# scaomath/galerkin-transformer

Measured on AMD Instinct MI355X. Metric: training samples/s, Darcy 141x141 Galerkin encoder (fwd+loss+bwd+clip+Adam), higher is better.
Workload: dtype f32 (operands split into 2 fp16 terms under a running per-row / per-tile power-of-two scale, 3 products on the f16 MFMA pipe, f32 accumulate; fp32-class results: the 1e-5 parity suite passes in this mode; packed-B token GEMMs, convolutions, weight gradients, regression head and the Fourier attention

## Files before the change

galerkin-transformer_amd/csrc/gt_head.hip:

```cpp
#include "gt_common.h"
#include <algorithm>

namespace gt {

constexpr int HK = 32, HN = 128;
constexpr int W1P = 36;
constexpr int DHP = 68;
constexpr int HSLAB = HN * HK + 2 * HN + 1;

struct HeadP {
    const float* X; const float* W1; const float* b1; const float* w2; const float* b2; const float* g;
    float* out; float* dX; float* slabs;
    int64_t T;
    int n_mtiles;
    const float* gate = nullptr;
};

__device__ __forceinline__ void head_gate4(const float* gp, f32x4& v) {
    const f32x4 gt = *reinterpret_cast<const f32x4*>(gp);
#pragma unroll
    for (int t = 0; t < 4; ++t) v[t] *= dsilu_f(gt[t]);
}

template <int ACT>
__device__ __forceinline__ void head_act(float h, float& a, float& da) {
    if (ACT == GT_ACT_SILU) silu_both(h, a, da);
    else if (ACT == GT_ACT_RELU) { a = fmaxf(h, 0.f); da = h > 0.f ? 1.f : 0.f; }
    else { a = h; da = 1.f; }
}

__device__ __forceinline__ void head_stage_weights(const HeadP& p, float* sW1, float* sB1, float* sW2) {
    const int tid = threadIdx.x;
    for (int e = tid; e < HN * HK; e += 256) sW1[(e >> 5) * W1P + (e & 31)] = p.W1[e];
    if (tid < HN) {
        sB1[tid] = p.b1 ? p.b1[tid] : 0.f;
        sW2[tid] = p.w2[tid];
    }
    __syncthreads();
}

template <int NMT>
__device__ __forceinline__ void head_gemm1(const float* sW1, int hb, int j, int kq, const float (&xs)[8],
                                           f32x4 (&acc)[NMT]) {
#pragma unroll
    for (int mt = 0; mt < NMT; mt += 2) {
        f32x4 w[2][2];
#pragma unroll
        for (int u = 0; u < 2; ++u) {
            w[u][0] = *reinterpret_cast<const f32x4*>(&sW1[(hb + 16 * (mt + u) + j) * W1P + 8 * kq]);
            w[u][1] = *reinterpret_cast<const f32x4*>(&sW1[(hb + 16 * (mt + u) + j) * W1P + 8 * kq + 4]);
            acc[mt + u] = f32x4{0.f, 0.f, 0.f, 0.f};
        }
#pragma unroll
        for (int s = 0; s < 8; ++s)
#pragma unroll
            for (int u = 0; u < 2; ++u)
                acc[mt + u] = __builtin_amdgcn_mfma_f32_16x16x4f32(w[u][s >> 2][s & 3], xs[s], acc[mt + u], 0, 0, 0);
    }
}

template <int ACT>
__global__ __launch_bounds__(256, 2) void head_fwd_kernel(const HeadP p) {
    __shared__ __attribute__((aligned(16))) float sW1[HN * W1P];
    __shared__ __attribute__((aligned(16))) float sB1[HN], sW2[HN];
    const int lane = threadIdx.x & 63, wave = threadIdx.x >> 6;
    const int j = lane & 15, kq = lane >> 4;
    head_stage_weights(p, sW1, sB1, sW2);
    const float b2v = p.b2 ? p.b2[0] : 0.f;
    const int stride = gridDim.x * 4;
    int mtile = blockIdx.x * 4 + wave;
    f32x4 xa = {0.f, 0.f, 0.f, 0.f}, xb = {0.f, 0.f, 0.f, 0.f};
    if (mtile < p.n_mtiles) {
        const int64_t row = std::min<int64_t>((int64_t)mtile * 16 + j, p.T - 1);
        xa = *reinterpret_cast<const f32x4*>(p.X + row * HK + 8 * kq);
        xb = *reinterpret_cast<const f32x4*>(p.X + row * HK + 8 * kq + 4);
    }
    for (; mtile < p.n_mtiles; mtile += stride) {
        const int64_t m0 = (int64_t)mtile * 16;
        const float xs[8] = {xa[0], xa[1], xa[2], xa[3], xb[0], xb[1], xb[2], xb[3]};
        if (mtile + stride < p.n_mtiles) {
            const int64_t row = std::min<int64_t>((int64_t)(mtile + stride) * 16 + j, p.T - 1);
            xa = *reinterpret_cast<const f32x4*>(p.X + row * HK + 8 * kq);
            xb = *reinterpret_cast<const f32x4*>(p.X + row * HK + 8 * kq + 4);
        }
        f32x4 acc[8];
        head_gemm1<8>(sW1, 0, j, kq, xs, acc);
        float part = 0.f;
#pragma unroll
        for (int mt = 0; mt < 8; ++mt) {
            const f32x4 bv = *reinterpret_cast<const f32x4*>(&sB1[16 * mt + 4 * kq]);
            const f32x4 wv = *reinterpret_cast<const f32x4*>(&sW2[16 * mt + 4 * kq]);
#pragma unroll
            for (int r = 0; r < 4; ++r) {
                float a, da;
                head_act<ACT>(acc[mt][r] + bv[r], a, da);
                part = fmaf(a, wv[r], part);
            }
        }
        part += __shfl_xor(part, 16, 64);
        part += __shfl_xor(part, 32, 64);
        if (kq == 0 && m0 + j < p.T) p.out[m0 + j] = part + b2v;
    }
}

template <int ACT>
__global__ __launch_bounds__(256, 2) void head_bwd_kernel(const HeadP p) {
    __shared__ __attribute__((aligned(16))) float sW1[HN * W1P];
    __shared__ __attribute__((aligned(16))) float sB1[HN], sW2[HN];
    __shared__ __attribute__((aligned(16))) float sScr[4 * 16 * DHP + 2 * 4 * 2 * 256];
    const int tid = threadIdx.x, lane = tid & 63, wave = tid >> 6;
    const int j = lane & 15, kq = lane >> 4;
    const int pair = wave >> 1, half = wave & 1, hb = 64 * half;
    head_stage_weights(p, sW1, sB1, sW2);
    float* dh = sScr + wave * 16 * DHP;
    float* exch = sScr + 4 * 16 * DHP;

    f32x4 accW[4][2], sumW2[4], sumB1[4];
    float gsum = 0.f;
#pragma unroll
    for (int mt = 0; mt < 4; ++mt) {
        accW[mt][0] = accW[mt][1] = f32x4{0.f, 0.f, 0.f, 0.f};
        sumW2[mt] = sumB1[mt] = f32x4{0.f, 0.f, 0.f, 0.f};
    }
    const int stride = gridDim.x * 2;
    const int first = blockIdx.x * 2;
    const int iters = first < p.n_mtiles ? (p.n_mtiles - 1 - first) / stride + 1 : 0;
    int mtile = first + pair;
    f32x4 xa = {0.f, 0.f, 0.f, 0.f}, xb = {0.f, 0.f, 0.f, 0.f};
    float gv = 0.f;
    if (mtile < p.n_mtiles) {
        const int64_t nrow = (int64_t)mtile * 16 + j, row = std::min<int64_t>(nrow, p.T - 1);
        xa = *reinterpret_cast<const f32x4*>(p.X + row * HK + 8 * kq);
        xb = *reinterpret_cast<const f32x4*>(p.X + row * HK + 8 * kq + 4);
        gv = (nrow < p.T) ? p.g[row] : 0.f;
    }
    for (int it = 0; it < iters; ++it, mtile += stride) {
        const bool active = mtile < p.n_mtiles;
        const int64_t m0 = (int64_t)mtile * 16;
        const float xs[8] = {xa[0], xa[1], xa[2], xa[3], xb[0], xb[1], xb[2], xb[3]};
        const float g = active ? gv : 0.f;
        if (mtile + stride < p.n_mtiles) {
            const int64_t nrow = (int64_t)(mtile + stride) * 16 + j, row = std::min<int64_t>(nrow, p.T - 1);
            xa = *reinterpret_cast<const f32x4*>(p.X + row * HK + 8 * kq);
            xb = *reinterpret_cast<const f32x4*>(p.X + row * HK + 8 * kq + 4);
            gv = (nrow < p.T) ? p.g[row] : 0.f;
        }
        float* ex = exch + (it & 1) * (4 * 2 * 256);
        f32x4 acc[4];
        f32x4 accX[2] = {{0.f, 0.f, 0.f, 0.f}, {0.f, 0.f, 0.f, 0.f}};
        if (active) {
            head_gemm1<4>(sW1, hb, j, kq, xs, acc);
            gsum += (kq == 0 && half == 0) ? g : 0.f;
#pragma unroll
            for (int mt = 0; mt < 4; ++mt) {
                const f32x4 bv = *reinterpret_cast<const f32x4*>(&sB1[hb + 16 * mt + 4 * kq]);
                const f32x4 wv = *reinterpret_cast<const f32x4*>(&sW2[hb + 16 * mt + 4 * kq]);
#pragma unroll
                for (int r = 0; r < 4; ++r) {
                    float a, da;
                    head_act<ACT>(acc[mt][r] + bv[r], a, da);
                    const float d = g * wv[r] * da;
                    sumW2[mt][r] = fmaf(g, a, sumW2[mt][r]);
                    sumB1[mt][r] += d;
                    acc[mt][r] = d;
                }
                *reinterpret_cast<f32x4*>(&dh[j * DHP + 16 * mt + 4 * kq]) = acc[mt];
            }
#pragma unroll
            for (int mt = 0; mt < 4; ++mt)
#pragma unroll
                for (int s = 0; s < 4; ++s)
#pragma unroll
                    for (int t = 0; t < 2; ++t)
                        accX[t] = __builtin_amdgcn_mfma_f32_16x16x4f32(
                            sW1[(hb + 16 * mt + 4 * kq + s) * W1P + 16 * t + j], acc[mt][s], accX[t], 0, 0, 0);
        }
        *reinterpret_cast<f32x4*>(&ex[(wave * 2 + (half ^ 1)) * 256 + lane * 4]) = accX[half ^ 1];
        __syncthreads();
        if (active) {
            if (p.dX && m0 + j < p.T) {
                const f32x4 o = *reinterpret_cast<const f32x4*>(&ex[((wave ^ 1) * 2 + half) * 256 + lane * 4]);
                f32x4 dxv = accX[half] + o;
                if (p.gate) head_gate4(p.gate + (m0 + j) * HK + 16 * half + 4 * kq, dxv);
                *reinterpret_cast<f32x4*>(p.dX + (m0 + j) * HK + 16 * half + 4 * kq) = dxv;
            }
            float xr[2][4];
#pragma unroll
            for (int s = 0; s < 4; ++s) {
                const int64_t row = std::min<int64_t>(m0 + 4 * kq + s, p.T - 1);
#pragma unroll
                for (int t = 0; t < 2; ++t) xr[t][s] = p.X[row * HK + 16 * t + j];
            }
#pragma unroll
            for (int mt = 0; mt < 4; ++mt)
#pragma unroll
                for (int s = 0; s < 4; ++s) {
                    const float a = dh[(4 * kq + s) * DHP + 16 * mt + j];
#pragma unroll
                    for (int t = 0; t < 2; ++t)
                        accW[mt][t] = __builtin_amdgcn_mfma_f32_16x16x4f32(a, xr[t][s], accW[mt][t], 0, 0, 0);
                }
        }
    }
#pragma unroll
    for (int mt = 0; mt < 4; ++mt)
#pragma unroll
        for (int r = 0; r < 4; ++r) {
            float a = sumW2[mt][r], b = sumB1[mt][r];
#pragma unroll
            for (int o = 1; o < 16; o <<= 1) {
                a += __shfl_xor(a, o, 64);
                b += __shfl_xor(b, o, 64);
            }
            sumW2[mt][r] = a;
            sumB1[mt][r] = b;
        }
#pragma unroll
    for (int o = 1; o < 16; o <<= 1) gsum += __shfl_xor(gsum, o, 64);
    __syncthreads();
    float* red = sScr;
    for (int w = 0; w < 4; ++w) {
        if (wave == w) {
            const bool init = w < 2;
#pragma unroll
            for (int mt = 0; mt < 4; ++mt) {
#pragma unroll
                for (int t = 0; t < 2; ++t)
#pragma unroll
                    for (int r = 0; r < 4; ++r) {
                        float* q = &red[(hb + 16 * mt + 4 * kq + r) * HK + 16 * t + j];
                        *q = init ? accW[mt][t][r] : *q + accW[mt][t][r];
                    }
                if (j == 0) {
#pragma unroll
                    for (int r = 0; r < 4; ++r) {
                        float* q2 = &red[HN * HK + hb + 16 * mt + 4 * kq + r];
                        float* q1 = &red[HN * HK + HN + hb + 16 * mt + 4 * kq + r];
                        *q2 = init ? sumW2[mt][r] : *q2 + sumW2[mt][r];
                        *q1 = init ? sumB1[mt][r] : *q1 + sumB1[mt][r];
                    }
                }
            }
            if (lane == 0 && half == 0) {
                float* q = &red[HN * HK + 2 * HN];
                *q = (w == 0) ? gsum : *q + gsum;
            }
        }
        __syncthreads();
    }
    float* out = p.slabs + (int64_t)blockIdx.x * HSLAB;
    for (int e = tid; e < HSLAB; e += 256) out[e] = red[e];
}

__global__ __launch_bounds__(256) void head_reduce_kernel(const float* __restrict__ slabs, int nslab, float* dW1,
                                                         float* dw2, float* db1, float* db2) {
    __shared__ float part[8][32];
    const int el = threadIdx.x & 31, sl = threadIdx.x >> 5;
    const int e = blockIdx.x * 32 + el;
    float a0 = 0.f, a1 = 0.f;
    if (e < HSLAB) {
        int s = sl;
        for (; s + 8 < nslab; s += 16) {
            a0 += slabs[(int64_t)s * HSLAB + e];
            a1 += slabs[(int64_t)(s + 8) * HSLAB + e];
        }
        if (s < nslab) a0 += slabs[(int64_t)s * HSLAB + e];
    }
    part[sl][el] = a0 + a1;
    __syncthreads();
    if (sl != 0 || e >= HSLAB) return;
    float v = part[0][el];
#pragma unroll
    for (int k = 1; k < 8; ++k) v += part[k][el];
    if (e < HN * HK) dW1[e] = v;
    else if (e < HN * HK + HN) { if (dw2) dw2[e - HN * HK] = v; }
    else if (e < HN * HK + 2 * HN) { if (db1) db1[e - HN * HK - HN] = v; }
    else if (db2) db2[0] = v;
}

typedef _Float16 hf16x8 __attribute__((ext_vector_type(8)));
typedef _Float16 hf16x2 __attribute__((ext_vector_type(2)));
typedef uint32_t hu32x4 __attribute__((ext_vector_type(4)));

__device__ __forceinline__ int h16_exp_for(float amax) {
    const int ex = (int)(__float_as_uint(amax) >> 23);
    return ex == 0 ? 0 : (141 - ex > 126 ? 126 : 141 - ex);
}
__device__ __forceinline__ void h16_split_pair(float a, float b, float s, uint32_t& hi, uint32_t& lo) {
    const f32x2 r = f32x2{a, b} * s;
    const hf16x2 h0 = __builtin_convertvector(r, hf16x2);
    const hf16x2 h1 = __builtin_convertvector(r - __builtin_convertvector(h0, f32x2), hf16x2);
    hi = __builtin_bit_cast(uint32_t, h0);
    lo = __builtin_bit_cast(uint32_t, h1);
}
__device__ __forceinline__ void h16_split8(const float (&v)[8], float s, hf16x8& hi, hf16x8& lo) {
    uint32_t h[4], l[4];
#pragma unroll
    for (int t = 0; t < 4; ++t) h16_split_pair(v[2 * t], v[2 * t + 1], s, h[t], l[t]);
    hi = __builtin_bit_cast(hf16x8, hu32x4{h[0], h[1], h[2], h[3]});
    lo = __builtin_bit_cast(hf16x8, hu32x4{l[0], l[1], l[2], l[3]});
}
__device__ __forceinline__ f32x4 h16_mma3(hf16x8 ah, hf16x8 al, hf16x8 bh, hf16x8 bl, f32x4 acc) {
    acc = __builtin_amdgcn_mfma_f32_16x16x32_f16(al, bh, acc, 0, 0, 0);
    acc = __builtin_amdgcn_mfma_f32_16x16x32_f16(ah, bl, acc, 0, 0, 0);
    return __builtin_amdgcn_mfma_f32_16x16x32_f16(ah, bh, acc, 0, 0, 0);
}

template <bool WT>
__device__ __forceinline__ int head16_stage(const HeadP& p, hu32x4* sW1, hu32x4* sWT, float* sB1, float* sW2, float* sRed) {
    const int tid = threadIdx.x, lane = tid & 63, wave = tid >> 6;
    float v[2][8], m = 0.f;
#pragma unroll
    for (int u = 0; u < 2; ++u) {
        const int f = tid + 256 * u, mt = f >> 6, j = f & 15, kq = (f & 63) >> 4;
        const f32x4 a = *reinterpret_cast<const f32x4*>(p.W1 + (16 * mt + j) * HK + 8 * kq);
        const f32x4 b = *reinterpret_cast<const f32x4*>(p.W1 + (16 * mt + j) * HK + 8 * kq + 4);
#pragma unroll
        for (int e = 0; e < 4; ++e) {
            v[u][e] = a[e];
            v[u][4 + e] = b[e];
            m = fmaxf(m, fmaxf(fabsf(a[e]), fabsf(b[e])));
        }
    }
#pragma unroll
    for (int o = 32; o > 0; o >>= 1) m = fmaxf(m, __shfl_xor(m, o, 64));
    if (lane == 0) sRed[wave] = m;
    if (tid < HN) {
        sB1[tid] = p.b1 ? p.b1[tid] : 0.f;
        sW2[tid] = p.w2[tid];
    }
    __syncthreads();
    const int eW = h16_exp_for(fmaxf(fmaxf(sRed[0], sRed[1]), fmaxf(sRed[2], sRed[3])));
    const float sw = pow2_clamped(eW);
#pragma unroll
    for (int u = 0; u < 2; ++u) {
        hf16x8 hi, lo;
        h16_split8(v[u], sw, hi, lo);
        sW1[tid + 256 * u] = __builtin_bit_cast(hu32x4, hi);
        sW1[512 + tid + 256 * u] = __builtin_bit_cast(hu32x4, lo);
    }
    if (WT) {
#pragma unroll
        for (int u = 0; u < 2; ++u) {
            const int f = tid + 256 * u, t = f >> 7, ti = (f >> 6) & 1, mm = f & 15, kq = (f & 63) >> 4;
            float w[8];
#pragma unroll
            for (int e = 0; e < 8; ++e) w[e] = p.W1[(32 * t + 16 * (e >> 2) + 4 * kq + (e & 3)) * HK + 16 * ti + mm];
            hf16x8 hi, lo;
            h16_split8(w, sw, hi, lo);
            sWT[f] = __builtin_bit_cast(hu32x4, hi);
            sWT[512 + f] = __builtin_bit_cast(hu32x4, lo);
        }
    }
    __syncthreads();
    return eW;
}

__device__ __forceinline__ int head16_split_row(const float (&xs)[8], hf16x8& xh, hf16x8& xl) {
    float m = 0.f;
#pragma unroll
    for (int e = 0; e < 8; ++e) m = fmaxf(m, fabsf(xs[e]));
    m = fmaxf(m, __shfl_xor(m, 16, 64));
    m = fmaxf(m, __shfl_xor(m, 32, 64));
    const int ex = h16_exp_for(m);
    h16_split8(xs, pow2_clamped(ex), xh, xl);
    return ex;
}

template <int ACT>
__global__ __launch_bounds__(256, 2) void head_fwd16_kernel(const HeadP p) {
    __shared__ hu32x4 sW1[2 * 512];
    __shared__ __attribute__((aligned(16))) float sB1[HN], sW2[HN];
    __shared__ float sRed[4];
    const int lane = threadIdx.x & 63, wave = threadIdx.x >> 6;
    const int j = lane & 15, kq = lane >> 4;
    const int eW = head16_stage<false>(p, sW1, nullptr, sB1, sW2, sRed);
    const float b2v = p.b2 ? p.b2[0] : 0.f;
    const int stride = gridDim.x * 4;
    int mtile = blockIdx.x * 4 + wave;
    f32x4 xa = {0.f, 0.f, 0.f, 0.f}, xb = {0.f, 0.f, 0.f, 0.f};
    if (mtile < p.n_mtiles) {
        const int64_t row = std::min<int64_t>((int64_t)mtile * 16 + j, p.T - 1);
        xa = *reinterpret_cast<const f32x4*>(p.X + row * HK + 8 * kq);
        xb = *reinterpret_cast<const f32x4*>(p.X + row * HK + 8 * kq + 4);
    }
    for (; mtile < p.n_mtiles; mtile += stride) {
        const int64_t m0 = (int64_t)mtile * 16;
        const float xs[8] = {xa[0], xa[1], xa[2], xa[3], xb[0], xb[1], xb[2], xb[3]};
        if (mtile + stride < p.n_mtiles) {
            const int64_t row = std::min<int64_t>((int64_t)(mtile + stride) * 16 + j, p.T - 1);
            xa = *reinterpret_cast<const f32x4*>(p.X + row * HK + 8 * kq);
            xb = *reinterpret_cast<const f32x4*>(p.X + row * HK + 8 * kq + 4);
        }
        hf16x8 xh, xl;
        const int ex = head16_split_row(xs, xh, xl);
        const float us = pow2_clamped(-ex) * pow2_clamped(-eW);
        float part = 0.f;
#pragma unroll
        for (int mt = 0; mt < 8; ++mt) {
            const hf16x8 wh = __builtin_bit_cast(hf16x8, sW1[mt * 64 + lane]);
            const hf16x8 wl = __builtin_bit_cast(hf16x8, sW1[512 + mt * 64 + lane]);
            const f32x4 acc = h16_mma3(wh, wl, xh, xl, f32x4{0.f, 0.f, 0.f, 0.f});
            const f32x4 bv = *reinterpret_cast<const f32x4*>(&sB1[16 * mt + 4 * kq]);
            const f32x4 wv = *reinterpret_cast<const f32x4*>(&sW2[16 * mt + 4 * kq]);
#pragma unroll
            for (int r = 0; r < 4; ++r) {
                float a, da;
                head_act<ACT>(fmaf(acc[r], us, bv[r]), a, da);
                part = fmaf(a, wv[r], part);
            }
        }
        part += __shfl_xor(part, 16, 64);
        part += __shfl_xor(part, 32, 64);
        if (kq == 0 && m0 + j < p.T) p.out[m0 + j] = part + b2v;
    }
}

constexpr int DH16P = 68;
constexpr int H16_LIMIT = 15, H16_TARGET = 13;
constexpr int H16_SMEM = 4 * 512 * 16 + (2 * HN + 16) * 4 + 4 * 32 * DH16P * 4 + 4 * 32 * 4 + 4 * 2 * 256 * 4;

template <int ACT>
__global__ __launch_bounds__(256, 2) void head_bwd16_kernel(const HeadP p) {
    extern __shared__ __attribute__((aligned(16))) char hsm[];
    hu32x4* sW1 = reinterpret_cast<hu32x4*>(hsm);
    hu32x4* sWT = sW1 + 1024;
    float* sB1 = reinterpret_cast<float*>(sWT + 1024);
    float* sW2 = sB1 + HN;
    float* sRed = sW2 + HN;
    float* sDh = sRed + 16;
    float* sF = sDh + 4 * 32 * DH16P;
    float* sEx = sF + 4 * 32;
    const int tid = threadIdx.x, lane = tid & 63, wave = tid >> 6;
    const int j = lane & 15, kq = lane >> 4;
    const int pair = wave >> 1, half = wave & 1, hb = 64 * half;
    const int eW = head16_stage<true>(p, sW1, sWT, sB1, sW2, sRed);
    const float usW = pow2_clamped(-eW);
    float* dh = sDh + wave * 32 * DH16P;
    float* fr = sF + wave * 32;

    f32x4 accW[4][2], sumW2[4], sumB1[4];
    float gsum = 0.f;
#pragma unroll
    for (int mt = 0; mt < 4; ++mt) {
        accW[mt][0] = accW[mt][1] = f32x4{0.f, 0.f, 0.f, 0.f};
        sumW2[mt] = sumB1[mt] = f32x4{0.f, 0.f, 0.f, 0.f};
    }
    int cexp = 100;
    const int n32 = (int)((p.T + 31) / 32);
    const int stride = gridDim.x * 2;
    const int first = blockIdx.x * 2;
    const int iters = first < n32 ? (n32 - 1 - first) / stride + 1 : 0;
    int tile = first + pair;
    f32x4 xa[2], xb[2];
    float gv[2];
    auto load = [&](int tl) {
#pragma unroll
        for (int u = 0; u < 2; ++u) {
            const int64_t nrow = (int64_t)tl * 32 + 16 * u + j, row = std::min<int64_t>(nrow, p.T - 1);
            xa[u] = *reinterpret_cast<const f32x4*>(p.X + row * HK + 8 * kq);
            xb[u] = *reinterpret_cast<const f32x4*>(p.X + row * HK + 8 * kq + 4);
            gv[u] = (nrow < p.T) ? p.g[row] : 0.f;
        }
    };
#pragma unroll
    for (int u = 0; u < 2; ++u) {
        xa[u] = xb[u] = f32x4{0.f, 0.f, 0.f, 0.f};
        gv[u] = 0.f;
    }
    if (tile < n32) load(tile);
    for (int it = 0; it < iters; ++it, tile += stride) {
        const bool active = tile < n32;
        const int64_t m0 = (int64_t)tile * 32;
        hf16x8 xh[2], xl[2];
        float us[2], xm[2], g[2];
#pragma unroll
        for (int u = 0; u < 2; ++u) {
            const float xs[8] = {xa[u][0], xa[u][1], xa[u][2], xa[u][3], xb[u][0], xb[u][1], xb[u][2], xb[u][3]};
            float m = 0.f;
#pragma unroll
            for (int e = 0; e < 8; ++e) m = fmaxf(m, fabsf(xs[e]));
            m = fmaxf(m, __shfl_xor(m, 16, 64));
            m = fmaxf(m, __shfl_xor(m, 32, 64));
            const int ex = h16_exp_for(m);
            h16_split8(xs, pow2_clamped(ex), xh[u], xl[u]);
            us[u] = pow2_clamped(-ex) * usW;
            xm[u] = m;
            g[u] = active ? gv[u] : 0.f;
        }
        if (tile + stride < n32) load(tile + stride);
        f32x4 own[2] = {{0.f, 0.f, 0.f, 0.f}, {0.f, 0.f, 0.f, 0.f}};
        float rowmag[2] = {0.f, 0.f};
        int edh[2] = {100000, 100000};
#pragma unroll
        for (int u = 0; u < 2; ++u) {
            f32x4 accX[2] = {{0.f, 0.f, 0.f, 0.f}, {0.f, 0.f, 0.f, 0.f}};
            if (active) {
                gsum += (kq == 0 && half == 0) ? g[u] : 0.f;
                float d[4][4], dm = 0.f;
#pragma unroll
                for (int mt = 0; mt < 4; ++mt) {
                    const int ft = (hb >> 4) + mt;
                    const hf16x8 wh = __builtin_bit_cast(hf16x8, sW1[ft * 64 + lane]);
                    const hf16x8 wl = __builtin_bit_cast(hf16x8, sW1[512 + ft * 64 + lane]);
                    const f32x4 acc = h16_mma3(wh, wl, xh[u], xl[u], f32x4{0.f, 0.f, 0.f, 0.f});
                    const f32x4 bv = *reinterpret_cast<const f32x4*>(&sB1[hb + 16 * mt + 4 * kq]);
                    const f32x4 wv = *reinterpret_cast<const f32x4*>(&sW2[hb + 16 * mt + 4 * kq]);
#pragma unroll
                    for (int r = 0; r < 4; ++r) {
                        float a, da;
                        head_act<ACT>(fmaf(acc[r], us[u], bv[r]), a, da);
                        const float dv = g[u] * wv[r] * da;
                        sumW2[mt][r] = fmaf(g[u], a, sumW2[mt][r]);
                        sumB1[mt][r] += dv;
                        d[mt][r] = dv;
                        dm = fmaxf(dm, fabsf(dv));
                    }
                }
                dm = fmaxf(dm, __shfl_xor(dm, 16, 64));
                dm = fmaxf(dm, __shfl_xor(dm, 32, 64));
                const int ed = h16_exp_for(dm);
                const float sd = pow2_clamped(ed);
                const bool live = (__float_as_uint(dm) >> 23) != 0;
                edh[u] = live ? ed : 100000;
                rowmag[u] = live ? xm[u] * pow2_clamped(-ed) : 0.f;
#pragma unroll
                for (int mt = 0; mt < 4; ++mt) {
#pragma unroll
                    for (int r = 0; r < 4; ++r) d[mt][r] *= sd;
                    *reinterpret_cast<f32x4*>(&dh[(16 * u + j) * DH16P + 16 * mt + 4 * kq]) =
                        f32x4{d[mt][0], d[mt][1], d[mt][2], d[mt][3]};
                }
#pragma unroll
                for (int t = 0; t < 2; ++t) {
                    const float dv8[8] = {d[2 * t][0], d[2 * t][1], d[2 * t][2], d[2 * t][3],
                                          d[2 * t + 1][0], d[2 * t + 1][1], d[2 * t + 1][2], d[2 * t + 1][3]};
                    hf16x8 dhi, dlo;
                    h16_split8(dv8, 1.f, dhi, dlo);
#pragma unroll
                    for (int ti = 0; ti < 2; ++ti) {
                        const int f = ((2 * half + t) * 2 + ti) * 64 + lane;
                        const hf16x8 wh = __builtin_bit_cast(hf16x8, sWT[f]);
                        const hf16x8 wl = __builtin_bit_cast(hf16x8, sWT[512 + f]);
                        accX[ti] = h16_mma3(wh, wl, dhi, dlo, accX[ti]);
                    }
                }
                const float ux = pow2_clamped(-ed) * usW;
                accX[0] *= ux;
                accX[1] *= ux;
            }
            *reinterpret_cast<f32x4*>(&sEx[(wave * 2 + u) * 256 + lane * 4]) = half ? accX[0] : accX[1];
            own[u] = half ? accX[1] : accX[0];
        }
        float xr[2][8];
#pragma unroll
        for (int e = 0; e < 8; ++e) {
            const int64_t row = std::min<int64_t>(m0 + 8 * kq + e, p.T - 1);
#pragma unroll
            for (int ti = 0; ti < 2; ++ti) xr[ti][e] = active ? p.X[row * HK + 16 * ti + j] : 0.f;
        }
        __syncthreads();
        if (active && p.dX) {
#pragma unroll
            for (int u = 0; u < 2; ++u)
                if (m0 + 16 * u + j < p.T) {
                    const f32x4 o = *reinterpret_cast<const f32x4*>(&sEx[((wave ^ 1) * 2 + u) * 256 + lane * 4]);
                    f32x4 dxv = own[u] + o;
                    if (p.gate) head_gate4(p.gate + (m0 + 16 * u + j) * HK + 16 * half + 4 * kq, dxv);
                    *reinterpret_cast<f32x4*>(p.dX + (m0 + 16 * u + j) * HK + 16 * half + 4 * kq) = dxv;
                }
        }
        if (active) {
            float mag = fmaxf(rowmag[0], rowmag[1]);
#pragma unroll
            for (int o = 1; o < 16; o <<= 1) mag = fmaxf(mag, __shfl_xor(mag, o, 64));
            const int xe = (int)(__float_as_uint(mag) >> 23);
            if (xe != 0 && xe + cexp - 127 >= H16_LIMIT) {
                const int cn = H16_TARGET + 127 - xe, dlt = cn - cexp;
                const float f = dlt < -126 ? 0.f : pow2_clamped(dlt);
#pragma unroll
                for (int mt = 0; mt < 4; ++mt) {
                    accW[mt][0] *= f;
                    accW[mt][1] *= f;
                }
                cexp = cn;
            }
            if (kq == 0) {
#pragma unroll
                for (int u = 0; u < 2; ++u) {
                    const int fe = cexp - edh[u];
                    fr[16 * u + j] = fe < -126 ? 0.f : pow2_clamped(fe);
                }
            }
            const f32x4 f0 = *reinterpret_cast<const f32x4*>(&fr[8 * kq]);
            const f32x4 f1 = *reinterpret_cast<const f32x4*>(&fr[8 * kq + 4]);
            const float fv[8] = {f0[0], f0[1], f0[2], f0[3], f1[0], f1[1], f1[2], f1[3]};
            hf16x8 bh[2], bl[2];
#pragma unroll
            for (int ti = 0; ti < 2; ++ti) {
                float w[8];
#pragma unroll
                for (int e = 0; e < 8; ++e) w[e] = xr[ti][e] * fv[e];
                h16_split8(w, 1.f, bh[ti], bl[ti]);
            }
#pragma unroll
            for (int mt = 0; mt < 4; ++mt) {
                float a8[8];
#pragma unroll
                for (int e = 0; e < 8; ++e) a8[e] = dh[(8 * kq + e) * DH16P + 16 * mt + j];
                hf16x8 ah, al;
                h16_split8(a8, 1.f, ah, al);
#pragma unroll
                for (int ti = 0; ti < 2; ++ti) accW[mt][ti] = h16_mma3(ah, al, bh[ti], bl[ti], accW[mt][ti]);
            }
        }
        __syncthreads();
    }
    {
        const float uc = pow2_clamped(-cexp);
#pragma unroll
        for (int mt = 0; mt < 4; ++mt) {
            accW[mt][0] *= uc;
            accW[mt][1] *= uc;
        }
    }
#pragma unroll
    for (int mt = 0; mt < 4; ++mt)
#pragma unroll
        for (int r = 0; r < 4; ++r) {
            float a = sumW2[mt][r], b = sumB1[mt][r];
#pragma unroll
            for (int o = 1; o < 16; o <<= 1) {
                a += __shfl_xor(a, o, 64);
                b += __shfl_xor(b, o, 64);
            }
            sumW2[mt][r] = a;
            sumB1[mt][r] = b;
        }
#pragma unroll
    for (int o = 1; o < 16; o <<= 1) gsum += __shfl_xor(gsum, o, 64);
    __syncthreads();
    float* red = sDh;
    for (int w = 0; w < 4; ++w) {
        if (wave == w) {
            const bool init = w < 2;
#pragma unroll
            for (int mt = 0; mt < 4; ++mt) {
#pragma unroll
                for (int t = 0; t < 2; ++t)
#pragma unroll
                    for (int r = 0; r < 4; ++r) {
                        float* q = &red[(hb + 16 * mt + 4 * kq + r) * HK + 16 * t + j];
                        *q = init ? accW[mt][t][r] : *q + accW[mt][t][r];
                    }
                if (j == 0) {
#pragma unroll
                    for (int r = 0; r < 4; ++r) {
                        float* q2 = &red[HN * HK + hb + 16 * mt + 4 * kq + r];
                        float* q1 = &red[HN * HK + HN + hb + 16 * mt + 4 * kq + r];
                        *q2 = init ? sumW2[mt][r] : *q2 + sumW2[mt][r];
                        *q1 = init ? sumB1[mt][r] : *q1 + sumB1[mt][r];
                    }
                }
            }
            if (lane == 0 && half == 0) {
                float* q = &red[HN * HK + 2 * HN];
                *q = (w == 0) ? gsum : *q + gsum;
            }
        }
        __syncthreads();
    }
    float* out = p.slabs + (int64_t)blockIdx.x * HSLAB;
    for (int e = tid; e < HSLAB; e += 256) out[e] = red[e];
}

static int head_blocks(int64_t T, int tiles_per_block) {
    const int64_t mt = (T + 15) / 16;
    return (int)std::min<int64_t>(512, (mt + tiles_per_block - 1) / tiles_per_block);
}

}

using namespace gt;

static int head_check(const float* X, int64_t T, int32_t K, int32_t N, int32_t n_out, const float* W1, const float* w2,
                      int32_t act) {
    if (!X || !W1 || !w2 || T <= 0) return GT_EINVAL;
    if (act != GT_ACT_NONE && act != GT_ACT_RELU && act != GT_ACT_SILU) return GT_EINVAL;
    if (K != HK || N != HN || n_out != 1 || T > (int64_t)1 << 34) return GT_ENOTSUP;
    if (reinterpret_cast<uintptr_t>(X) & 15) return GT_EALIGN;
    return 0;
}

static bool head_use_f16(int32_t precision) { return precision == GT_PREC_F16X2; }

extern "C" int gt_mlp_head_fwd(const float* X, int64_t T, int32_t K, int32_t N, int32_t n_out, const float* W1,
                               const float* b1, const float* w2, const float* b2, int32_t act, int32_t precision,
                               float* out, void* stream) {
    int rc = head_check(X, T, K, N, n_out, W1, w2, act);
    if (rc) return rc;
    if (!out || precision < GT_PREC_F32 || precision > GT_PREC_F16X2) return GT_EINVAL;
    HeadP p{X, W1, b1, w2, b2, nullptr, out, nullptr, nullptr, T, (int)((T + 15) / 16)};
    dim3 grid((unsigned)head_blocks(T, 4));
    hipStream_t st = (hipStream_t)stream;
    if (head_use_f16(precision)) {
        if (act == GT_ACT_SILU) hipLaunchKernelGGL((head_fwd16_kernel<GT_ACT_SILU>), grid, dim3(256), 0, st, p);
        else if (act == GT_ACT_RELU) hipLaunchKernelGGL((head_fwd16_kernel<GT_ACT_RELU>), grid, dim3(256), 0, st, p);
        else hipLaunchKernelGGL((head_fwd16_kernel<GT_ACT_NONE>), grid, dim3(256), 0, st, p);
        GT_LAUNCH_CHECK();
        return 0;
    }
    if (act == GT_ACT_SILU) hipLaunchKernelGGL((head_fwd_kernel<GT_ACT_SILU>), grid, dim3(256), 0, st, p);
    else if (act == GT_ACT_RELU) hipLaunchKernelGGL((head_fwd_kernel<GT_ACT_RELU>), grid, dim3(256), 0, st, p);
    else hipLaunchKernelGGL((head_fwd_kernel<GT_ACT_NONE>), grid, dim3(256), 0, st, p);
    GT_LAUNCH_CHECK();
    return 0;
}

extern "C" int64_t gt_mlp_head_bwd_ws_bytes(int64_t T) {
    return T > 0 ? (int64_t)head_blocks(T, 2) * HSLAB * (int64_t)sizeof(float) : 0;
}

extern "C" int gt_mlp_head_bwd(const float* X, int64_t T, int32_t K, int32_t N, int32_t n_out, const float* W1,
                               const float* b1, const float* w2, int32_t act, int32_t precision, const float* g,
                               float* dX, float* dW1, float* db1, float* dw2, float* db2, void* ws, int64_t ws_bytes,
                               void* stream) {
    return gt_mlp_head_bwd_gated(X, T, K, N, n_out, W1, b1, w2, act, precision, g, dX, nullptr, dW1, db1, dw2, db2, ws,
                                 ws_bytes, stream);
}

extern "C" int gt_mlp_head_bwd_gated(const float* X, int64_t T, int32_t K, int32_t N, int32_t n_out, const float* W1,
                                     const float* b1, const float* w2, int32_t act, int32_t precision, const float* g,
                                     float* dX, const float* dx_gate, float* dW1, float* db1, float* dw2, float* db2,
                                     void* ws, int64_t ws_bytes, void* stream) {
    int rc = head_check(X, T, K, N, n_out, W1, w2, act);
    if (rc) return rc;
    if (dx_gate && !dX) return GT_EINVAL;
    if (reinterpret_cast<uintptr_t>(dx_gate) & 15) return GT_EALIGN;
    if (!g || !dW1 || precision < GT_PREC_F32 || precision > GT_PREC_F16X2) return GT_EINVAL;
    if (reinterpret_cast<uintptr_t>(dX) & 15) return GT_EALIGN;
    if (!ws || ws_bytes < gt_mlp_head_bwd_ws_bytes(T)) return GT_EWS;
    hipStream_t st = (hipStream_t)stream;
    if (head_use_f16(precision)) {
        const int64_t n32 = (T + 31) / 32;
        const int blocks16 = (int)std::min<int64_t>(512, (n32 + 1) / 2);
        HeadP q{X, W1, b1, w2, nullptr, g, nullptr, dX, reinterpret_cast<float*>(ws), T, (int)((T + 15) / 16), dx_gate};
        if (gt_allow_dynamic_lds<head_bwd16_kernel<GT_ACT_NONE>>(H16_SMEM) ||
            gt_allow_dynamic_lds<head_bwd16_kernel<GT_ACT_RELU>>(H16_SMEM) ||
            gt_allow_dynamic_lds<head_bwd16_kernel<GT_ACT_SILU>>(H16_SMEM))
            return GT_ENOTSUP;
        if (act == GT_ACT_SILU)
            hipLaunchKernelGGL((head_bwd16_kernel<GT_ACT_SILU>), dim3(blocks16), dim3(256), H16_SMEM, st, q);
        else if (act == GT_ACT_RELU)
            hipLaunchKernelGGL((head_bwd16_kernel<GT_ACT_RELU>), dim3(blocks16), dim3(256), H16_SMEM, st, q);
        else hipLaunchKernelGGL((head_bwd16_kernel<GT_ACT_NONE>), dim3(blocks16), dim3(256), H16_SMEM, st, q);
        GT_LAUNCH_CHECK();
        hipLaunchKernelGGL(head_reduce_kernel, dim3((HSLAB + 31) / 32), dim3(256), 0, st, reinterpret_cast<const float*>(ws),
                           blocks16, dW1, dw2, db1, db2);
        GT_LAUNCH_CHECK();
        return 0;
    }
    const int blocks = head_blocks(T, 2);
    HeadP p{X, W1, b1, w2, nullptr, g, nullptr, dX, reinterpret_cast<float*>(ws), T, (int)((T + 15) / 16), dx_gate};
    if (act == GT_ACT_SILU) hipLaunchKernelGGL((head_bwd_kernel<GT_ACT_SILU>), dim3(blocks), dim3(256), 0, st, p);
    else if (act == GT_ACT_RELU) hipLaunchKernelGGL((head_bwd_kernel<GT_ACT_RELU>), dim3(blocks), dim3(256), 0, st, p);
    else hipLaunchKernelGGL((head_bwd_kernel<GT_ACT_NONE>), dim3(blocks), dim3(256), 0, st, p);
    GT_LAUNCH_CHECK();
    hipLaunchKernelGGL(head_reduce_kernel, dim3((HSLAB + 31) / 32), dim3(256), 0, st, reinterpret_cast<const float*>(ws),
                       blocks, dW1, dw2, db1, db2);
    GT_LAUNCH_CHECK();
    return 0;
}
```

Baseline: 6222.

## Restructure fp16-split MLP head backward: 512-thread blocks, pre-split dh tiles, LDS X transpose

The head backward kernel moves to 512-thread blocks with four 32-row tile pairs per block, and is templated on dX/gate so those branches are resolved at compile time. It stores the gradient tile to LDS already split into packed fp16 hi/lo pairs, and stages an X transpose in LDS instead of re-reading strided global X for the weight-gradient MFMA. Cross-lane reductions switch to permlane16_swap and DPP row ops in place of shuffles. Forward launch bounds and grid size are also retuned. The goal is less redundant global traffic and conversion work, at the cost of more LDS, one block per CU, and occupancy risk.

```diff
diff --git a/galerkin-transformer_amd/csrc/gt_head.hip b/galerkin-transformer_amd/csrc/gt_head.hip
--- a/galerkin-transformer_amd/csrc/gt_head.hip
+++ b/galerkin-transformer_amd/csrc/gt_head.hip
@@ -282,6 +282,27 @@
 typedef _Float16 hf16x2 __attribute__((ext_vector_type(2)));
 typedef uint32_t hu32x4 __attribute__((ext_vector_type(4)));
 
+__device__ __forceinline__ float kq_max(float v) {
+    const uint32_t u = __float_as_uint(v);
+    const auto sw = __builtin_amdgcn_permlane16_swap(u, u, false, false);
+    return xor32_max(fmaxf(__uint_as_float(sw[0]), __uint_as_float(sw[1])));
+}
+__device__ __forceinline__ float kq_sum(float v) {
+    const uint32_t u = __float_as_uint(v);
+    const auto sw = __builtin_amdgcn_permlane16_swap(u, u, false, false);
+    return xor32_sum(__uint_as_float(sw[0]) + __uint_as_float(sw[1]));
+}
+template <int CTRL>
+__device__ __forceinline__ float dpp_row(float v) {
+    return __int_as_float(__builtin_amdgcn_update_dpp(0, __float_as_int(v), CTRL, 0xf, 0xf, true));
+}
+__device__ __forceinline__ float row16_max(float v) {
+    v = fmaxf(v, dpp_row<0x128>(v));
+    v = fmaxf(v, dpp_row<0x124>(v));
+    v = fmaxf(v, dpp_row<0x122>(v));
+    return fmaxf(v, dpp_row<0x121>(v));
+}
+
 __device__ __forceinline__ int h16_exp_for(float amax) {
     const int ex = (int)(__float_as_uint(amax) >> 23);
     return ex == 0 ? 0 : (141 - ex > 126 ? 126 : 141 - ex);
@@ -306,13 +327,14 @@
     return __builtin_amdgcn_mfma_f32_16x16x32_f16(ah, bh, acc, 0, 0, 0);
 }
 
-template <bool WT>
+template <bool WT, int NT>
 __device__ __forceinline__ int head16_stage(const HeadP& p, hu32x4* sW1, hu32x4* sWT, float* sB1, float* sW2, float* sRed) {
+    constexpr int NU = 512 / NT;
     const int tid = threadIdx.x, lane = tid & 63, wave = tid >> 6;
-    float v[2][8], m = 0.f;
-#pragma unroll
-    for (int u = 0; u < 2; ++u) {
-        const int f = tid + 256 * u, mt = f >> 6, j = f & 15, kq = (f & 63) >> 4;
+    float v[NU][8], m = 0.f;
+#pragma unroll
+    for (int u = 0; u < NU; ++u) {
+        const int f = tid + NT * u, mt = f >> 6, j = f & 15, kq = (f & 63) >> 4;
         const f32x4 a = *reinterpret_cast<const f32x4*>(p.W1 + (16 * mt + j) * HK + 8 * kq);
         const f32x4 b = *reinterpret_cast<const f32x4*>(p.W1 + (16 * mt + j) * HK + 8 * kq + 4);
 #pragma unroll
@@ -330,19 +352,22 @@
         sW2[tid] = p.w2[tid];
     }
     __syncthreads();
-    const int eW = h16_exp_for(fmaxf(fmaxf(sRed[0], sRed[1]), fmaxf(sRed[2], sRed[3])));
+    float mw = sRed[0];
+#pragma unroll
+    for (int w = 1; w < NT / 64; ++w) mw = fmaxf(mw, sRed[w]);
+    const int eW = h16_exp_for(mw);
     const float sw = pow2_clamped(eW);
 #pragma unroll
-    for (int u = 0; u < 2; ++u) {
+    for (int u = 0; u < NU; ++u) {
         hf16x8 hi, lo;
         h16_split8(v[u], sw, hi, lo);
-        sW1[tid + 256 * u] = __builtin_bit_cast(hu32x4, hi);
-        sW1[512 + tid + 256 * u] = __builtin_bit_cast(hu32x4, lo);
+        sW1[tid + NT * u] = __builtin_bit_cast(hu32x4, hi);
+        sW1[512 + tid + NT * u] = __builtin_bit_cast(hu32x4, lo);
     }
     if (WT) {
 #pragma unroll
-        for (int u = 0; u < 2; ++u) {
-            const int f = tid + 256 * u, t = f >> 7, ti = (f >> 6) & 1, mm = f & 15, kq = (f & 63) >> 4;
+        for (int u = 0; u < NU; ++u) {
+            const int f = tid + NT * u, t = f >> 7, ti = (f >> 6) & 1, mm = f & 15, kq = (f & 63) >> 4;
             float w[8];
 #pragma unroll
             for (int e = 0; e < 8; ++e) w[e] = p.W1[(32 * t + 16 * (e >> 2) + 4 * kq + (e & 3)) * HK + 16 * ti + mm];
@@ -360,21 +385,20 @@
     float m = 0.f;
 #pragma unroll
     for (int e = 0; e < 8; ++e) m = fmaxf(m, fabsf(xs[e]));
-    m = fmaxf(m, __shfl_xor(m, 16, 64));
-    m = fmaxf(m, __shfl_xor(m, 32, 64));
+    m = kq_max(m);
     const int ex = h16_exp_for(m);
     h16_split8(xs, pow2_clamped(ex), xh, xl);
     return ex;
 }
 
 template <int ACT>
-__global__ __launch_bounds__(256, 2) void head_fwd16_kernel(const HeadP p) {
+__global__ __launch_bounds__(256, 3) void head_fwd16_kernel(const HeadP p) {
     __shared__ hu32x4 sW1[2 * 512];
     __shared__ __attribute__((aligned(16))) float sB1[HN], sW2[HN];
     __shared__ float sRed[4];
     const int lane = threadIdx.x & 63, wave = threadIdx.x >> 6;
     const int j = lane & 15, kq = lane >> 4;
-    const int eW = head16_stage<false>(p, sW1, nullptr, sB1, sW2, sRed);
+    const int eW = head16_stage<false, 256>(p, sW1, nullptr, sB1, sW2, sRed);
     const float b2v = p.b2 ? p.b2[0] : 0.f;
     const int stride = gridDim.x * 4;
     int mtile = blockIdx.x * 4 + wave;
@@ -410,33 +434,41 @@
                 part = fmaf(a, wv[r], part);
             }
         }
-        part += __shfl_xor(part, 16, 64);
-        part += __shfl_xor(part, 32, 64);
+        part = kq_sum(part);
         if (kq == 0 && m0 + j < p.T) p.out[m0 + j] = part + b2v;
     }
 }
 
-constexpr int DH16P = 68;
+constexpr int H16_NT = 512;
+constexpr int DH16P = 36;
+constexpr int XT16P = 36;
 constexpr int H16_LIMIT = 15, H16_TARGET = 13;
-constexpr int H16_SMEM = 4 * 512 * 16 + (2 * HN + 16) * 4 + 4 * 32 * DH16P * 4 + 4 * 32 * 4 + 4 * 2 * 256 * 4;
-
-template <int ACT>
-__global__ __launch_bounds__(256, 2) void head_bwd16_kernel(const HeadP p) {
-    extern __shared__ __attribute__((aligned(16))) char hsm[];
+constexpr int H16_SMEM = 4 * 512 * 16 + (2 * HN + 16) * 4 + 8 * 64 * DH16P * 4 + 4 * 32 * XT16P * 4 + 8 * 32 * 4 +
+                         8 * 2 * 256 * 4;
+
+__device__ __forceinline__ void h16_zip(uint32_t a, uint32_t b, uint32_t& w0, uint32_t& w1) {
+    w0 = __builtin_amdgcn_perm(b, a, 0x05040100u);
+    w1 = __builtin_amdgcn_perm(b, a, 0x07060302u);
+}
+
+template <int ACT, bool DX, bool GATE>
+__device__ __forceinline__ void head_bwd16_body(const HeadP& p, char* hsm) {
     hu32x4* sW1 = reinterpret_cast<hu32x4*>(hsm);
     hu32x4* sWT = sW1 + 1024;
     float* sB1 = reinterpret_cast<float*>(sWT + 1024);
     float* sW2 = sB1 + HN;
     float* sRed = sW2 + HN;
-    float* sDh = sRed + 16;
-    float* sF = sDh + 4 * 32 * DH16P;
-    float* sEx = sF + 4 * 32;
+    uint32_t* sDh = reinterpret_cast<uint32_t*>(sRed + 16);
+    float* sXT = reinterpret_cast<float*>(sDh + 8 * 64 * DH16P);
+    float* sF = sXT + 4 * 32 * XT16P;
+    float* sEx = sF + 8 * 32;
     const int tid = threadIdx.x, lane = tid & 63, wave = tid >> 6;
     const int j = lane & 15, kq = lane >> 4;
     const int pair = wave >> 1, half = wave & 1, hb = 64 * half;
-    const int eW = head16_stage<true>(p, sW1, sWT, sB1, sW2, sRed);
+    const int eW = head16_stage<true, H16_NT>(p, sW1, sWT, sB1, sW2, sRed);
     const float usW = pow2_clamped(-eW);
-    float* dh = sDh + wave * 32 * DH16P;
+    uint32_t* dh = sDh + wave * 64 * DH16P;
+    float* xt = sXT + pair * 32 * XT16P;
     float* fr = sF + wave * 32;
 
     f32x4 accW[4][2], sumW2[4], sumB1[4];
@@ -448,27 +480,22 @@
     }
     int cexp = 100;
     const int n32 = (int)((p.T + 31) / 32);
-    const int stride = gridDim.x * 2;
-    const int first = blockIdx.x * 2;
+    const int stride = gridDim.x * 4;
+    const int first = blockIdx.x * 4;
     const int iters = first < n32 ? (n32 - 1 - first) / stride + 1 : 0;
     int tile = first + pair;
-    f32x4 xa[2], xb[2];
+    f32x4 xa[2], xb[2], gq[2];
     float gv[2];
     auto load = [&](int tl) {
 #pragma unroll
         for (int u = 0; u < 2; ++u) {
-            const int64_t nrow = (int64_t)tl * 32 + 16 * u + j, row = std::min<int64_t>(nrow, p.T - 1);
+            const int64_t row = std::min<int64_t>((int64_t)tl * 32 + 16 * u + j, p.T - 1);
             xa[u] = *reinterpret_cast<const f32x4*>(p.X + row * HK + 8 * kq);
             xb[u] = *reinterpret_cast<const f32x4*>(p.X + row * HK + 8 * kq + 4);
-            gv[u] = (nrow < p.T) ? p.g[row] : 0.f;
+            gv[u] = p.g[row];
         }
     };
-#pragma unroll
-    for (int u = 0; u < 2; ++u) {
-        xa[u] = xb[u] = f32x4{0.f, 0.f, 0.f, 0.f};
-        gv[u] = 0.f;
-    }
-    if (tile < n32) load(tile);
+    load(tile);
     for (int it = 0; it < iters; ++it, tile += stride) {
         const bool active = tile < n32;
         const int64_t m0 = (int64_t)tile * 32;
@@ -480,15 +507,29 @@
             float m = 0.f;
 #pragma unroll
             for (int e = 0; e < 8; ++e) m = fmaxf(m, fabsf(xs[e]));
-            m = fmaxf(m, __shfl_xor(m, 16, 64));
-            m = fmaxf(m, __shfl_xor(m, 32, 64));
+            m = kq_max(m);
             const int ex = h16_exp_for(m);
             h16_split8(xs, pow2_clamped(ex), xh[u], xl[u]);
             us[u] = pow2_clamped(-ex) * usW;
             xm[u] = m;
-            g[u] = active ? gv[u] : 0.f;
-        }
-        if (tile + stride < n32) load(tile + stride);
+            g[u] = (active && m0 + 16 * u + j < p.T) ? gv[u] : 0.f;
+        }
+        {
+            const f32x4 wa = half ? xa[1] : xa[0], wb = half ? xb[1] : xb[0];
+#pragma unroll
+            for (int e = 0; e < 4; ++e) {
+                xt[(8 * kq + e) * XT16P + 16 * half + j] = wa[e];
+                xt[(8 * kq + 4 + e) * XT16P + 16 * half + j] = wb[e];
+            }
+        }
+        if (GATE) {
+#pragma unroll
+            for (int u = 0; u < 2; ++u) {
+                const int64_t row = std::min<int64_t>(m0 + 16 * u + j, p.T - 1);
+                gq[u] = *reinterpret_cast<const f32x4*>(p.gate + row * HK + 16 * half + 4 * kq);
+            }
+        }
+        load(tile + stride);
         f32x4 own[2] = {{0.f, 0.f, 0.f, 0.f}, {0.f, 0.f, 0.f, 0.f}};
         float rowmag[2] = {0.f, 0.f};
         int edh[2] = {100000, 100000};
@@ -517,63 +558,70 @@
                         dm = fmaxf(dm, fabsf(dv));
                     }
                 }
-                dm = fmaxf(dm, __shfl_xor(dm, 16, 64));
-                dm = fmaxf(dm, __shfl_xor(dm, 32, 64));
+                dm = kq_max(dm);
                 const int ed = h16_exp_for(dm);
                 const float sd = pow2_clamped(ed);
                 const bool live = (__float_as_uint(dm) >> 23) != 0;
                 edh[u] = live ? ed : 100000;
                 rowmag[u] = live ? xm[u] * pow2_clamped(-ed) : 0.f;
 #pragma unroll
-                for (int mt = 0; mt < 4; ++mt) {
+                for (int mt = 0; mt < 4; ++mt)
 #pragma unroll
                     for (int r = 0; r < 4; ++r) d[mt][r] *= sd;
-                    *reinterpret_cast<f32x4*>(&dh[(16 * u + j) * DH16P + 16 * mt + 4 * kq]) =
-                        f32x4{d[mt][0], d[mt][1], d[mt][2], d[mt][3]};
-                }
 #pragma unroll
                 for (int t = 0; t < 2; ++t) {
                     const float dv8[8] = {d[2 * t][0], d[2 * t][1], d[2 * t][2], d[2 * t][3],
                                           d[2 * t + 1][0], d[2 * t + 1][1], d[2 * t + 1][2], d[2 * t + 1][3]};
                     hf16x8 dhi, dlo;
                     h16_split8(dv8, 1.f, dhi, dlo);
-#pragma unroll
-                    for (int ti = 0; ti < 2; ++ti) {
-                        const int f = ((2 * half + t) * 2 + ti) * 64 + lane;
-                        const hf16x8 wh = __builtin_bit_cast(hf16x8, sWT[f]);
-                        const hf16x8 wl = __builtin_bit_cast(hf16x8, sWT[512 + f]);
-                        accX[ti] = h16_mma3(wh, wl, dhi, dlo, accX[ti]);
+                    const hu32x4 hw = __builtin_bit_cast(hu32x4, dhi), lw = __builtin_bit_cast(hu32x4, dlo);
+#pragma unroll
+                    for (int q = 0; q < 4; ++q) {
+                        uint32_t w0, w1;
+                        h16_zip(hw[q], lw[q], w0, w1);
+                        const int h0 = 32 * t + 16 * (q >> 1) + 4 * kq + 2 * (q & 1);
+                        dh[h0 * DH16P + 16 * u + j] = w0;
+                        dh[(h0 + 1) * DH16P + 16 * u + j] = w1;
+                    }
+                    if (DX) {
+#pragma unroll
+                        for (int ti = 0; ti < 2; ++ti) {
+                            const int f = ((2 * half + t) * 2 + ti) * 64 + lane;
+                            const hf16x8 wh = __builtin_bit_cast(hf16x8, sWT[f]);
+                            const hf16x8 wl = __builtin_bit_cast(hf16x8, sWT[512 + f]);
+                            accX[ti] = h16_mma3(wh, wl, dhi, dlo, accX[ti]);
+                        }
                     }
                 }
                 const float ux = pow2_clamped(-ed) * usW;
                 accX[0] *= ux;
                 accX[1] *= ux;
             }
-            *reinterpret_cast<f32x4*>(&sEx[(wave * 2 + u) * 256 + lane * 4]) = half ? accX[0] : accX[1];
-            own[u] = half ? accX[1] : accX[0];
-        }
-        float xr[2][8];
-#pragma unroll
-        for (int e = 0; e < 8; ++e) {
-            const int64_t row = std::min<int64_t>(m0 + 8 * kq + e, p.T - 1);
-#pragma unroll
-            for (int ti = 0; ti < 2; ++ti) xr[ti][e] = active ? p.X[row * HK + 16 * ti + j] : 0.f;
+            if (DX) {
+                *reinterpret_cast<f32x4*>(&sEx[(wave * 2 + u) * 256 + lane * 4]) = half ? accX[0] : accX[1];
+                own[u] = half ? accX[1] : accX[0];
+            }
         }
         __syncthreads();
-        if (active && p.dX) {
+        if (DX) {
+            f32x4 dxv[2];
+#pragma unroll
+            for (int u = 0; u < 2; ++u) {
+                const f32x4 o = *reinterpret_cast<const f32x4*>(&sEx[((wave ^ 1) * 2 + u) * 256 + lane * 4]);
+                dxv[u] = own[u] + o;
+                if (GATE) {
+#pragma unroll
+                    for (int t = 0; t < 4; ++t) dxv[u][t] *= dsilu_f(gq[u][t]);
+                }
+            }
+            asm volatile("" : "+v"(dxv[0]), "+v"(dxv[1]));
 #pragma unroll
             for (int u = 0; u < 2; ++u)
-                if (m0 + 16 * u + j < p.T) {
-                    const f32x4 o = *reinterpret_cast<const f32x4*>(&sEx[((wave ^ 1) * 2 + u) * 256 + lane * 4]);
-                    f32x4 dxv = own[u] + o;
-                    if (p.gate) head_gate4(p.gate + (m0 + 16 * u + j) * HK + 16 * half + 4 * kq, dxv);
-                    *reinterpret_cast<f32x4*>(p.dX + (m0 + 16 * u + j) * HK + 16 * half + 4 * kq) = dxv;
-                }
+                if (active && m0 + 16 * u + j < p.T)
+                    *reinterpret_cast<f32x4*>(p.dX + (m0 + 16 * u + j) * HK + 16 * half + 4 * kq) = dxv[u];
         }
         if (active) {
-            float mag = fmaxf(rowmag[0], rowmag[1]);
-#pragma unroll
-            for (int o = 1; o < 16; o <<= 1) mag = fmaxf(mag, __shfl_xor(mag, o, 64));
+            const float mag = row16_max(fmaxf(rowmag[0], rowmag[1]));
             const int xe = (int)(__float_as_uint(mag) >> 23);
             if (xe != 0 && xe + cexp - 127 >= H16_LIMIT) {
                 const int cn = H16_TARGET + 127 - xe, dlt = cn - cexp;
@@ -598,18 +646,23 @@
             hf16x8 bh[2], bl[2];
 #pragma unroll
             for (int ti = 0; ti < 2; ++ti) {
-                float w[8];
-#pragma unroll
-                for (int e = 0; e < 8; ++e) w[e] = xr[ti][e] * fv[e];
+                const f32x4 x0 = *reinterpret_cast<const f32x4*>(&xt[(16 * ti + j) * XT16P + 8 * kq]);
+                const f32x4 x1 = *reinterpret_cast<const f32x4*>(&xt[(16 * ti + j) * XT16P + 8 * kq + 4]);
+                const float w[8] = {x0[0] * fv[0], x0[1] * fv[1], x0[2] * fv[2], x0[3] * fv[3],
+                                    x1[0] * fv[4], x1[1] * fv[5], x1[2] * fv[6], x1[3] * fv[7]};
                 h16_split8(w, 1.f, bh[ti], bl[ti]);
             }
 #pragma unroll
             for (int mt = 0; mt < 4; ++mt) {
-                float a8[8];
-#pragma unroll
-                for (int e = 0; e < 8; ++e) a8[e] = dh[(8 * kq + e) * DH16P + 16 * mt + j];
-                hf16x8 ah, al;
-                h16_split8(a8, 1.f, ah, al);
+                const hu32x4 a0 = *reinterpret_cast<const hu32x4*>(&dh[(16 * mt + j) * DH16P + 8 * kq]);
+                const hu32x4 a1 = *reinterpret_cast<const hu32x4*>(&dh[(16 * mt + j) * DH16P + 8 * kq + 4]);
+                uint32_t hw[4], lw[4];
+                h16_zip(a0[0], a0[1], hw[0], lw[0]);
+                h16_zip(a0[2], a0[3], hw[1], lw[1]);
+                h16_zip(a1[0], a1[1], hw[2], lw[2]);
+                h16_zip(a1[2], a1[3], hw[3], lw[3]);
+                const hf16x8 ah = __builtin_bit_cast(hf16x8, hu32x4{hw[0], hw[1], hw[2], hw[3]});
+                const hf16x8 al = __builtin_bit_cast(hf16x8, hu32x4{lw[0], lw[1], lw[2], lw[3]});
 #pragma unroll
                 for (int ti = 0; ti < 2; ++ti) accW[mt][ti] = h16_mma3(ah, al, bh[ti], bl[ti], accW[mt][ti]);
             }
@@ -640,8 +693,8 @@
 #pragma unroll
     for (int o = 1; o < 16; o <<= 1) gsum += __shfl_xor(gsum, o, 64);
     __syncthreads();
-    float* red = sDh;
-    for (int w = 0; w < 4; ++w) {
+    float* red = reinterpret_cast<float*>(sDh);
+    for (int w = 0; w < H16_NT / 64; ++w) {
         if (wave == w) {
             const bool init = w < 2;
 #pragma unroll
@@ -671,7 +724,15 @@
         __syncthreads();
     }
     float* out = p.slabs + (int64_t)blockIdx.x * HSLAB;
-    for (int e = tid; e < HSLAB; e += 256) out[e] = red[e];
+    for (int e = tid; e < HSLAB; e += H16_NT) out[e] = red[e];
+}
+
+template <int ACT>
+__global__ __launch_bounds__(H16_NT, 1) void head_bwd16_kernel(const HeadP p) {
+    extern __shared__ __attribute__((aligned(16))) char hsm[];
+    if (p.gate) head_bwd16_body<ACT, true, true>(p, hsm);
+    else if (p.dX) head_bwd16_body<ACT, true, false>(p, hsm);
+    else head_bwd16_body<ACT, false, false>(p, hsm);
 }
 
 static int head_blocks(int64_t T, int tiles_per_block) {
@@ -704,6 +765,7 @@
     dim3 grid((unsigned)head_blocks(T, 4));
     hipStream_t st = (hipStream_t)stream;
     if (head_use_f16(precision)) {
+        grid = dim3((unsigned)std::min<int64_t>(768, ((T + 15) / 16 + 3) / 4));
         if (act == GT_ACT_SILU) hipLaunchKernelGGL((head_fwd16_kernel<GT_ACT_SILU>), grid, dim3(256), 0, st, p);
         else if (act == GT_ACT_RELU) hipLaunchKernelGGL((head_fwd16_kernel<GT_ACT_RELU>), grid, dim3(256), 0, st, p);
         else hipLaunchKernelGGL((head_fwd16_kernel<GT_ACT_NONE>), grid, dim3(256), 0, st, p);
@@ -743,17 +805,17 @@
     hipStream_t st = (hipStream_t)stream;
     if (head_use_f16(precision)) {
         const int64_t n32 = (T + 31) / 32;
-        const int blocks16 = (int)std::min<int64_t>(512, (n32 + 1) / 2);
+        const int blocks16 = (int)std::min<int64_t>(256, (n32 + 3) / 4);
         HeadP q{X, W1, b1, w2, nullptr, g, nullptr, dX, reinterpret_cast<float*>(ws), T, (int)((T + 15) / 16), dx_gate};
         if (gt_allow_dynamic_lds<head_bwd16_kernel<GT_ACT_NONE>>(H16_SMEM) ||
             gt_allow_dynamic_lds<head_bwd16_kernel<GT_ACT_RELU>>(H16_SMEM) ||
             gt_allow_dynamic_lds<head_bwd16_kernel<GT_ACT_SILU>>(H16_SMEM))
             return GT_ENOTSUP;
         if (act == GT_ACT_SILU)
-            hipLaunchKernelGGL((head_bwd16_kernel<GT_ACT_SILU>), dim3(blocks16), dim3(256), H16_SMEM, st, q);
+            hipLaunchKernelGGL((head_bwd16_kernel<GT_ACT_SILU>), dim3(blocks16), dim3(H16_NT), H16_SMEM, st, q);
         else if (act == GT_ACT_RELU)
-            hipLaunchKernelGGL((head_bwd16_kernel<GT_ACT_RELU>), dim3(blocks16), dim3(256), H16_SMEM, st, q);
-        else hipLaunchKernelGGL((head_bwd16_kernel<GT_ACT_NONE>), dim3(blocks16), dim3(256), H16_SMEM, st, q);
+            hipLaunchKernelGGL((head_bwd16_kernel<GT_ACT_RELU>), dim3(blocks16), dim3(H16_NT), H16_SMEM, st, q);
+        else hipLaunchKernelGGL((head_bwd16_kernel<GT_ACT_NONE>), dim3(blocks16), dim3(H16_NT), H16_SMEM, st, q);
         GT_LAUNCH_CHECK();
         hipLaunchKernelGGL(head_reduce_kernel, dim3((HSLAB + 31) / 32), dim3(256), 0, st, reinterpret_cast<const float*>(ws),
                            blocks16, dW1, dw2, db1, db2);
```

Measured after the change: 6252 (median of 6 runs). No clear change (+0.5%).
